# wildjames/lfit_python

Measured on AMD Instinct MI355X. Metric: walker ln_prob evals/sec (300-pt phase, complex BS) at 1/2/4/8 MI355X, higher is better.
Workload: dtype f64

## Files before the change

### cpu_baseline/cpu.py

```python
import ctypes
import os
import subprocess

import numpy as np

HERE = os.path.dirname(os.path.abspath(__file__))
ROOT = os.path.dirname(HERE)
LIB_PATH = os.path.join(HERE, "liblfg_cpu.so")
_dp = ctypes.POINTER(ctypes.c_double)
_ip = ctypes.POINTER(ctypes.c_int)


def build(out=None, march="x86-64-v3"):
    out = out or LIB_PATH
    cmd = ["g++", "-O3", "-march=%s" % march, "-fopenmp", "-std=c++17", "-fPIC", "-shared",
           "-I", HERE, "-I", os.path.join(HERE, "shim"), "-I", os.path.join(ROOT, "lfit_python_amd", "csrc"),
           "-I", os.path.join(ROOT, "include"), "-o", out, os.path.join(HERE, "lfg_cpu.cpp")]
    subprocess.run(cmd, check=True)
    return out


class CpuPort:
    def __init__(self, path=None):
        self.lib = ctypes.CDLL(path or LIB_PATH)
        f = self.lib.lfc_lnprob_batch
        f.restype = ctypes.c_int
        f.argtypes = [_dp, ctypes.c_int, ctypes.c_int, ctypes.c_int, _ip, _ip, _dp, _ip, _dp, _dp, _dp, _dp,
                      ctypes.c_int, _ip, _dp, _dp, _dp, ctypes.c_int, _dp, ctypes.c_int]
        for name in ("lfg_cpu_flux", "lfg_cpu_lnlike", "lfg_cpu_lnprob"):
            getattr(self.lib, name).restype = ctypes.c_int
        self.lib.lfg_cpu_flux.argtypes = [_dp, ctypes.c_int, ctypes.c_int, _dp, _dp, ctypes.c_int, ctypes.c_int,
                                          _dp, _ip, ctypes.c_int]
        self.lib.lfg_cpu_lnlike.argtypes = [_dp, ctypes.c_int, ctypes.c_int, _dp, _dp, ctypes.c_int, ctypes.c_int,
                                            _dp, _dp, _dp, _ip, ctypes.c_int]
        g = self.lib.lfc_lnprob_batch_gp
        g.restype = ctypes.c_int
        g.argtypes = [_dp, ctypes.c_int, ctypes.c_int, ctypes.c_int, _ip, _ip, _dp, _ip, _dp, _dp, _dp, _dp,
                      ctypes.c_int, _ip, _dp, _dp, _dp, ctypes.c_int, _ip, _dp, _ip, _dp, ctypes.c_int]

    def lnprob_batch(self, walkers, tree, nthreads=0):
        keep = []

        def F(a):
            a = np.ascontiguousarray(a, dtype=np.float64)
            keep.append(a)
            return a.ctypes.data_as(_dp)

        def I(a):
            a = np.ascontiguousarray(a, dtype=np.int32)
            keep.append(a)
            return a.ctypes.data_as(_ip)
        w = np.ascontiguousarray(walkers, dtype=np.float64)
        W, ndim = w.shape
        lnp = np.empty(W)
        gp = bool(getattr(tree, "gp", False))
        used = self.lib.lfc_lnprob_batch_gp(
            F(w), W, ndim, tree.E, I(tree.gather.reshape(-1)), I(tree.npars),
            F(tree.consts if len(tree.consts) else np.zeros(1)), I(tree.offsets), F(tree.x), F(tree.y), F(tree.ye),
            F(tree.w), int(tree.nsub), I(tree.prior_type), F(tree.prior_p1), F(tree.prior_p2), F(tree.prior_norm),
            int(tree.roche_priors), I(tree.gp_gather.reshape(-1)) if gp else None,
            F(tree.gp_base.reshape(-1)) if gp else None, I(tree.gp_ecl.reshape(-1)) if gp else None,
            lnp.ctypes.data_as(_dp), int(nthreads))
        if getattr(tree, "fixed_invalid", False):
            lnp[:] = -np.inf
        return lnp, used

    def flux(self, pars, x, w, nsub=1, nthreads=0):
        pars = np.ascontiguousarray(np.atleast_2d(pars), dtype=np.float64)
        x = np.ascontiguousarray(x, dtype=np.float64)
        w = None if w is None else np.ascontiguousarray(w, dtype=np.float64)
        W, P = pars.shape
        flux = np.empty((W, x.size))
        st = np.empty(W, dtype=np.int32)
        rc = self.lib.lfg_cpu_flux(pars.ctypes.data_as(_dp), W, P, x.ctypes.data_as(_dp),
                                   None if w is None else w.ctypes.data_as(_dp), x.size, int(nsub),
                                   flux.ctypes.data_as(_dp), st.ctypes.data_as(_ip), int(nthreads))
        if rc != 0:
            raise ValueError("lfg_cpu_flux: code %d" % rc)
        return flux, st

    def lnlike(self, pars, x, w, y, ye, nsub=1, nthreads=0):
        pars = np.ascontiguousarray(np.atleast_2d(pars), dtype=np.float64)
        arr = [np.ascontiguousarray(a, dtype=np.float64) for a in (x, y, ye)]
        w = None if w is None else np.ascontiguousarray(w, dtype=np.float64)
        W, P = pars.shape
        out = np.empty(W)
        st = np.empty(W, dtype=np.int32)
        rc = self.lib.lfg_cpu_lnlike(pars.ctypes.data_as(_dp), W, P, arr[0].ctypes.data_as(_dp),
                                     None if w is None else w.ctypes.data_as(_dp), arr[0].size, int(nsub),
                                     arr[1].ctypes.data_as(_dp), arr[2].ctypes.data_as(_dp), out.ctypes.data_as(_dp),
                                     st.ctypes.data_as(_ip), int(nthreads))
        if rc != 0:
            raise ValueError("lfg_cpu_lnlike: code %d" % rc)
        return out, st

    def gp_predict(self, x, ye, obs, res, hyp, blocks, return_var=True, nthreads=0):
        x, ye = (np.ascontiguousarray(a, dtype=np.float64).reshape(-1) for a in (x, ye))
        obs = np.ascontiguousarray(obs, dtype=np.int32).reshape(-1)
# ... 48 lines not shown
```

### cpu_baseline/lfg_cpu.cpp

```cpp
#include <omp.h>
#include <stdint.h>
#include <stdlib.h>

#include <algorithm>
#include <cmath>
#include <vector>

#include "lfg.h"
#include "lfg_cpu.h"
#include "lfg_device.hpp"
#include "lfg_tables.hpp"

using namespace lfg;

namespace {

constexpr int U_WD = NWD / 2, U_DISC = NDISC / 2, U_DON = NDONOR / 4;

struct Pair {
    Roche R;
    double s, c, rwd_a, rdisc_a, reff, rcal, ulimb, dexp, L, upk, umax, lnpk, exp1, exp2;
    double bsx, bsy, caz, saz, nb0, nb1, nb2, bden, fis, phi0, wdf, df, sf, rsf;
    double inc;
};
// ... 38 lines not shown
    if (st == ST_OK && (!(p[9] > 0.0) || !(p[14] > 0.0) || !(p[15] > 0.0))) st = ST_BAD_GEOMETRY;
    double bs[4] = {0.0, 0.0, 0.0, 0.0};
    int bst = (std::isfinite(p[6]) && std::isfinite(p[10])) ? bspot<false>(R, G.rdisc_a, bs, &qp) : ST_BAD_ARGS;
    if (bst != ST_OK) {
        rprior = -INFINITY;
    } else {
        double alpha = std::atan2(bs[1], bs[0]) / DEG;
        if (alpha < 0.0) alpha = 90.0 - alpha;
        const double tangent = alpha + 90.0;
        if (p[10] < std::fmax(0.0, tangent - AZ_SLOPE) || p[10] > std::fmin(178.0, tangent + AZ_SLOPE)) rprior = -INFINITY;
    }
    if (st != ST_OK) return st;
    if (bst != ST_OK) return bst;
    const double a1 = p[14], a2 = p[15];
    G.upk = std::pow(a1 / a2, 1.0 / a2);
    G.lnpk = a1 * std::log(G.upk) - std::pow(G.upk, a2);
    G.umax = bs_umax(a1, a2, G.lnpk);
    if (!(std::isfinite(G.upk) && std::isfinite(G.lnpk) && std::isfinite(G.umax))) return ST_BAD_GEOMETRY;
    G.exp1 = a1;
    G.exp2 = a2;
    G.bsx = bs[0];
    G.bsy = bs[1];
    G.s = std::sin(inc * DEG);
    G.c = std::cos(inc * DEG);
    const double tilt = p[16] * DEG, psi = (p[10] - 90.0 + p[17]) * DEG;
    const double st_ = std::sin(tilt), ct_ = std::cos(tilt);
    G.nb0 = st_ * std::cos(psi);
    G.nb1 = st_ * std::sin(psi);
    G.nb2 = ct_;
    G.caz = std::cos(p[10] * DEG);
    G.saz = std::sin(p[10] * DEG);
    G.bden = p[11] + (1.0 - p[11]) * std::fmax(std::fabs(st_) * G.s + ct_ * G.c, 0.0);
    G.fis = p[11];
    G.phi0 = p[13];
    G.ulimb = p[7];
    G.dexp = p[12];
    G.L = p[9] * R.xl1;
    G.reff = eggleton(R.q);
    const double sce = G.s * std::cos(PI * p[5]);
    G.rcal = std::sqrt(1.0 - sce * sce);
    G.wdf = p[0]; G.df = p[1]; G.sf = p[2]; G.rsf = p[3];
    G.inc = inc;
    return ST_OK;
}

struct Tables {
    double a[NWD + NDISC], b[NWD + NDISC], w[NWD + NDISC];
    int wd[NWD + NDISC];
    double sa[NBS], sb[NBS], sw[NBS];
    double dv[NDONOR][3], dcen[NDONOR], dhw[NDONOR];
    double dnorm;
};

#ifdef LFC_COUNT
static unsigned long long g_cnt[4 + 3 * 8];
extern "C" void lfc_counts(unsigned long long* o) { for (int i = 0; i < 4 + 24; ++i) o[i] = g_cnt[i]; }
static unsigned long long g_ucost[U_WD + U_DISC + NBS];
extern "C" void lfc_ucost(unsigned long long* o) { for (int i = 0; i < U_WD + U_DISC + NBS; ++i) { o[i] = g_ucost[i]; g_ucost[i] = 0; } }
static void count_pair(const int* cost, int n)
{
    unsigned long long ls = 0, cm = 0, nc = 0;
    for (int k = 0; k < n; k += 64) {
        int m = 0;
        for (int i = k; i < std::min(n, k + 64); ++i) {
            m = std::max(m, cost[i]);
            ls += cost[i];
            const int reg = i < U_WD ? 0 : (i < U_WD + U_DISC ? 1 : 2);
#pragma omp atomic
            g_ucost[i] += cost[i];
#pragma omp atomic
            g_cnt[4 + reg * 8 + std::min(cost[i], 7)] += 1;
        }
        cm += m; ++nc;
    }
#pragma omp atomic
    g_cnt[0] += n;
#pragma omp atomic
    g_cnt[1] += ls;
#pragma omp atomic
    g_cnt[2] += nc;
#pragma omp atomic
    g_cnt[3] += cm;
}
#define LFC_NIT int nit[3] = {0, 0, 0}; bool fb = false; double gs[2] = {0.0, 0.0};
#define LFC_NITARGS , &fb, nit, gs
#if LFC_COST_MODE == 1
#define LFC_COST(v) cost[v] = nit[0] / 1000
#elif LFC_COST_MODE == 2
#define LFC_COST(v) cost[v] = nit[0] % 1000 + std::max(nit[1], nit[2]) + (fb ? 30 : 0)
#else
#define LFC_COST(v) cost[v] = nit[0] + std::max(nit[1], nit[2]) + (fb ? 30 : 0)
#endif
static std::vector<double> g_ab;
extern "C" long lfc_dump(double* o, long n)
{
    const long m = std::min<long>(n, long(g_ab.size()));
    for (long i = 0; i < m; ++i) o[i] = g_ab[i];
    g_ab.clear();
    return m;
}
#define LFC_AB(a, b) do { _Pragma("omp critical") { g_ab.push_back(a); g_ab.push_back(b); g_gs.push_back(gs[0]); g_gs.push_back(gs[1]); } } while (0)
static std::vector<double> g_gs;
extern "C" long lfc_dump_guess(double* o, long n)
{
    const long m = std::min<long>(n, long(g_gs.size()));
    for (long i = 0; i < m; ++i) o[i] = g_gs[i];
    g_gs.clear();
    return m;
}
#else
#define LFC_NIT
#define LFC_NITARGS
#define LFC_COST(v)
#define LFC_AB(a, b)
#endif

void elements(const Pair& G, Tables& T)
{
#ifdef LFC_COUNT
    int cost[U_WD + U_DISC + NBS] = {0};
#endif
    const Roche& R = G.R;
    const double s = G.s, c = G.c;
    const double twd = TWO_PI * ((1.0 - G.ulimb) * 0.5 + G.ulimb / 3.0);
    const double td = TWO_PI * (disc_boundary(NDISC_R, G) - disc_boundary(0, G));
    int k = 0;
    for (int u = 0; u < U_WD + U_DISC; ++u) {
        double Px, Py, Pz, wgt;
        bool isw = u < U_WD;
        if (isw) {
            const int ir = wd_ring_of(u);
            const double rc = kWdRc[ir], mu0 = kWdMu0[ir], cp = kWdCos[u], sp = kWdSin[u];
            Px = G.rwd_a * (-rc * sp * c + mu0 * s);
            Py = G.rwd_a * (rc * cp);
            Pz = G.rwd_a * (rc * sp * s + mu0 * c);
            wgt = std::fma(kWdA[ir], 1.0 - G.ulimb, kWdB[ir] * G.ulimb) / twd;
        } else {
            const int uu = u - U_WD, ir = uu / (NDISC_AZ / 2), j = uu - ir * (NDISC_AZ / 2);
            const double rc = G.rwd_a + (ir + 0.5) * ((G.rdisc_a - G.rwd_a) / NDISC_R);
            Px = rc * kDiscCos[j];
            Py = rc * kDiscSin[j];
            Pz = 0.0;
            wgt = (TWO_PI / NDISC_AZ) * (disc_boundary(ir + 1, G) - disc_boundary(ir, G)) / td;
        }
        double a, b;
        LFC_NIT
        element_interval_fast(R, Px, Py, Pz, s, c, G.rcal, G.reff, a, b LFC_NITARGS);
        LFC_COST(u);
        LFC_AB(a, b);
        T.a[k] = a; T.b[k] = b; T.w[k] = wgt; T.wd[k] = isw; ++k;
        const bool ecl = a < b;
        T.a[k] = ecl ? -b : 1.0; T.b[k] = ecl ? -a : -1.0; T.w[k] = wgt; T.wd[k] = isw; ++k;
    }
    double tot = 0.0;
    for (int j = 0; j < NBS; ++j) {
        const double uk = (j + 0.5) * (G.umax / NBS);
        T.sw[j] = std::exp(G.exp1 * std::log(uk) - std::pow(uk, G.exp2) - G.lnpk);
        tot += T.sw[j];
        const double off = G.L * (uk - G.upk);
        LFC_NIT
        element_interval_fast(R, std::fma(off, G.caz, G.bsx), std::fma(off, G.saz, G.bsy), 0.0, s, c, G.rcal, G.reff,
                              T.sa[j], T.sb[j] LFC_NITARGS);
        LFC_COST(U_WD + U_DISC + j);
        LFC_AB(T.sa[j], T.sb[j]);
    }
#ifdef LFC_COUNT
    count_pair(cost, U_WD + U_DISC + NBS);
#endif
    for (int j = 0; j < NBS; ++j) T.sw[j] /= tot;
    double dn = 0.0;
    for (int uu = 0; uu < U_DON; ++uu) {
        const int it = uu / (NDONOR_P / 4), ip = uu - it * (NDONOR_P / 4);
        const double dx = -kDonCt[it], dy = kDonSt[it] * kDonCp[ip], dz = kDonSt[it] * kDonSp[ip];
        double lo = 0.0, hi = R.Rs, r = G.reff, gx, gy, gz;
        if (!(r > lo && r < hi)) r = 0.5 * hi;
        for (int itr = 0; itr < ROOT_MAXIT; ++itr) {
            const double f = rpot_grad(R, std::fma(r, dx, 1.0), r * dy, r * dz, gx, gy, gz) - R.pl1;
            const double df = gx * dx + gy * dy + gz * dz;
            if (f > 0.0) hi = r; else lo = r;
            if (df > 0.0 && std::fabs(f / df) <= ROOT_LAST) { r -= f / df; break; }
            double rn = (df > 0.0) ? r - f / df : 0.5 * (lo + hi);
            if (!(rn > lo && rn < hi)) rn = 0.5 * (lo + hi);
            r = rn;
        }
        rgrad(R, std::fma(r, dx, 1.0), r * dy, r * dz, gx, gy, gz);
        const double ig = 1.0 / std::sqrt(gx * gx + gy * gy + gz * gz);
        const double nx = gx * ig, ny = gy * ig, nz = gz * ig;
        const double dA = r * r * kDonOmega[it] / (nx * dx + ny * dy + nz * dz);
        const double vx = dA * nx, vy = dA * ny, vz = dA * nz;
        const double srho = s * std::sqrt(vx * vx + vy * vy);
        const double kap = (srho > 0.0) ? -c * vz / srho : (c * vz > 0.0 ? -2.0 : 2.0);
        const double cen = -std::atan2(vy, vx) / TWO_PI, hw = std::acos(std::fmin(std::fmax(kap, -1.0), 1.0)) / TWO_PI;
        for (int mr = 0; mr < 4; ++mr) {
            const int t = 4 * uu + mr;
            T.dv[t][0] = vx;
            T.dv[t][1] = (mr & 1) ? -vy : vy;
            T.dv[t][2] = (mr & 2) ? -vz : vz;
            T.dcen[t] = (mr & 1) ? -cen : cen;
            T.dhw[t] = (mr & 2) ? 0.5 - hw : hw;
            dn += std::fmax(-s * T.dv[t][1] + c * T.dv[t][2], 0.0);
        }
    }
    T.dnorm = dn;
}

double wrap_phase(double ph) { return ph - std::floor(ph + 0.5); }

void sweep_window(const double* lo, const double* hi, const double* iw, int m, double a, double b, double wn,
                  double* d, double* direct)
{
    const int P2 = int(std::lower_bound(lo, lo + m, a) - lo);
    const int P4 = int(std::lower_bound(lo, lo + m, b) - lo);
    const int P1 = int(std::upper_bound(hi, hi + m, a) - hi);
    const int P3 = int(std::upper_bound(hi, hi + m, b) - hi);
    int e0 = P4, s1 = P4;
    if (P2 < P3) {
        d[P2] += wn;
        d[P3] -= wn;
        e0 = P2;
        s1 = P3;
    }
    for (int r = 0; r < 2; ++r)
        for (int p = r ? s1 : P1; p < (r ? P4 : e0); ++p) {
            if (hi[p] > lo[p]) {
                const double ov = std::fmin(b, hi[p]) - std::fmax(a, lo[p]);
                if (ov > 0.0) direct[p] += wn * ov * iw[p];
            } else if (a < lo[p] && lo[p] < b) {
                direct[p] += wn;
            }
        }
}

void sweep_points(const double* ph, int m, double x1, double x2, const double* v, std::vector<double>& d3)
{
    const int P = int(std::upper_bound(ph, ph + m, x1) - ph), Q = int(std::lower_bound(ph, ph + m, x2) - ph);
    if (P < Q)
        for (int k = 0; k < 3; ++k) {
            d3[3 * P + k] += v[k];
            d3[3 * Q + k] -= v[k];
        }
}

double chisq(const Pair& G, const Tables& T, const double* x, const double* w, const double* y, const double* ye, int n,
             int S, std::vector<double>& buf, double* fout = nullptr)
{
    const int ns = n * S;
    buf.assign(size_t(9) * n + size_t(10) * ns + 8, 0.0);
    double* lo = buf.data();
    double* hi = lo + n;
    double* iw = hi + n;
    double* dw = iw + n;
    double* dd = dw + n + 1;
    double* xw = dd + n + 1;
    double* xd = xw + n;
    double* slo = xd + n + 1;
    double* shi = slo + ns;
    double* siw = shi + ns;
    double* sph = siw + ns;
    double* ds = sph + ns;
// ... 353 lines not shown
```

### cpu_baseline/shim/hip/hip_runtime.h

```cpp
#pragma once
#include <algorithm>
#include <cmath>
#define __device__
#define __host__
#define __global__
#define __constant__
#define __forceinline__ inline
#define __noinline__
#define __builtin_amdgcn_rsq(x) (1.0 / std::sqrt(x))
#define __builtin_amdgcn_rcp(x) (1.0 / (x))
using std::max;
using std::min;
inline double rsqrt(double x) { return 1.0 / std::sqrt(x); }
inline float rsqrtf(float x) { return 1.0f / std::sqrt(x); }
```

### lfit_python_amd/csrc/lfg.hip

```cpp
#include <hip/hip_runtime.h>
#include <atomic>
#include <stdint.h>
#include <stdlib.h>

#include <type_traits>

#include "lfg.h"
#include "lfg_device.hpp"
#include "lfg_tables.hpp"

using namespace lfg;

#if defined(LFG_PROFILE_PAIR) || defined(LFG_COUNT_ITERS) || defined(LFG_COUNT_QUIET)
#define LFG_ONE_TU 1
#endif

namespace {

constexpr int SETUP_BLOCK = 64;
#ifndef LFG_ELEM_BLOCK
#define LFG_ELEM_BLOCK 64
#endif
constexpr int ELEM_BLOCK = LFG_ELEM_BLOCK;
#ifndef LFG_ELEM_IPL
// ... 520 lines not shown
template <typename GPtr>
__device__ __forceinline__ void ring_weight_lane(int rb, GPtr G, double* __restrict__ wtd)
{
    const double P = disc_boundary(rb, G);
    const int lane = int(threadIdx.x) & 63, l0 = lane - rb;
    const double Pn = __shfl(P, min(lane + 1, l0 + NDISC_R), 64);
    const double Pt = __shfl(P, l0 + NDISC_R, 64);
    if (rb < NDISC_R) wtd[rb] = (TWO_PI / NDISC_AZ) * (Pn - P);
    if (rb == 0) wtd[NDISC_R] = TWO_PI * (Pt - P);
}

template <typename GPtr, typename Sink>
__device__ __forceinline__ void element_item_to(int v, GPtr G, Sink& K);

struct MemSink {
    const ElemOut& O;
    __device__ __forceinline__ void mark() {}
    __device__ __forceinline__ void wd_disc(int u, double a, double b) { O.abw[uslot(u)] = make_double2(a, b); }
    __device__ __forceinline__ void spot(int j, double a, double b, double w)
    {
        O.abs[j] = make_double2(a, b);
        O.wbs[j] = w;
    }
    __device__ __forceinline__ void donor(int uu, double vx, double vy, double vz, double cen, double hw)
    {
        double* D = O.don + uu * DON_STRIDE;
        D[0] = vx;
        D[1] = vy;
        D[2] = vz;
        D[3] = cen;
        D[4] = hw;
    }
};

template <typename GPtr>
__device__ __forceinline__ void element_item(int v, GPtr G, const ElemOut& O)
{
    MemSink K{O};
    element_item_to(v, G, K);
}

__device__ __forceinline__ void element_lane(int v, int pair, int npairs, const double* __restrict__ G, int st0, int bst,
                                             int* status, double2* __restrict__ AB, double* __restrict__ DON,
                                             double* __restrict__ WT, const ElemSpec& X)
{
    double* Wp = WT + size_t(pair) * WT_N;
    if (v >= NUNIQ) {
        const int rb = v - NUNIQ;
        if (rb > NDISC_R || st0 != ST_OK) return;
        ring_weight_lane(rb, G, Wp + WT_DISC);
        return;
    }
    static_assert((NUNIQ % ELEM_BLOCK) + NDISC_R + 1 <= ELEM_BLOCK, "ring-weight lanes fit in the last chunk");
    static_assert(WT_TD == WT_DISC + NDISC_R, "disc total follows the ring weights");
    if (st0 != ST_OK) return;
    if (bst != ST_OK) {
        if (v == 0 && !X.jk) status[pair] = bst;
        return;
    }
    if (X.lprior) {
        const int w = pair / X.E;
        const double lp = X.jk ? X.priorC[size_t(X.accflag[X.jk[w]]) * (npairs / X.E) + w] : X.lprior[w];
        if (prior_rejects(lp, G)) return;
    }
    double2* ABp = AB + size_t(pair) * NELU;
    element_item(v, G, ElemOut{ABp, ABp + NU_WDD, DON + size_t(pair) * U_DON * DON_STRIDE, Wp + WT_DISC, Wp + WT_BS});
}

template <typename GPtr, typename Sink>
__device__ __forceinline__ void element_item_to(int v, GPtr G, Sink& K)
{
    constexpr int V_BS = U_WD + U_DISC;
    const int u = (v < V_BS) ? v : (v < V_BS + U_BS ? U_MAIN + (v - V_BS) : v - U_BS);
    const Roche R{G[G_Q], G[G_CA], G[G_CB], G[G_MU], G[G_XL1], G[G_PL1], G[G_RS], G[G_RS2]};
    const double s = G[G_S], c = G[G_C];

    if (u >= U_WD + U_DISC && u < U_MAIN) {
        const int uu = u - (U_WD + U_DISC);
        const int it = uu / (NDONOR_P / 4), ip = uu - it * (NDONOR_P / 4);
        const double stc = kDonSt[it], ctc = kDonCt[it];
        const double dx = -ctc, dy = stc * kDonCp[ip], dz = stc * kDonSp[ip];
        double lo = 0.0, hi = R.Rs, r = G[G_REFF];
        if (!(r > lo && r < hi)) r = 0.5 * hi;
        double gx, gy, gz;
        for (int itr = 0; itr < ROOT_MAXIT; ++itr) {
            const double X0 = fma(r, dx, 1.0), X1 = r * dy, X2 = r * dz;
            const double f = rpot_grad(R, X0, X1, X2, gx, gy, gz) - R.pl1;
            const double df = gx * dx + gy * dy + gz * dz;
            if (f > 0.0) hi = r; else lo = r;
            const double stp = f * rcp_fast(df);
            if (df > 0.0 && fabs(stp) <= ROOT_LAST) { r -= stp; break; }
            double rn = (df > 0.0) ? r - stp : 0.5 * (lo + hi);
            if (!(rn > lo && rn < hi)) rn = 0.5 * (lo + hi);
            r = rn;
        }
        rgrad(R, fma(r, dx, 1.0), r * dy, r * dz, gx, gy, gz);
        const double ig = rsqrt(gx * gx + gy * gy + gz * gz);
        const double nx = gx * ig, ny = gy * ig, nz = gz * ig;
        const double dA = r * r * kDonOmega[it] / (nx * dx + ny * dy + nz * dz);
        const double vx = dA * nx, vy = dA * ny, vz = dA * nz;
        const double srho = s * sqrt(vx * vx + vy * vy);
        const double kap = (srho > 0.0) ? -c * vz / srho : (c * vz > 0.0 ? -2.0 : 2.0);
        const double cen = -atan2(vy, vx) * (1.0 / TWO_PI), hw = acos(fmin(fmax(kap, -1.0), 1.0)) * (1.0 / TWO_PI);
        K.mark();
        K.donor(uu, vx, vy, vz, cen, hw);
        return;
    }

    double Px, Py, Pz;
    if (u < U_WD) {
        const int ir = wd_ring_of(u);
        const double rc = kWdRc[ir], mu0 = kWdMu0[ir];
        const double cp = kWdCos[u], sp = kWdSin[u];
        const double rw = G[G_RWD];
        Px = rw * (-rc * sp * c + mu0 * s);
        Py = rw * (rc * cp);
        Pz = rw * (rc * sp * s + mu0 * c);
    } else if (u < U_WD + U_DISC) {
        const int uu = u - U_WD;
        const int ir = uu / (NDISC_AZ / 2), j = uu - ir * (NDISC_AZ / 2);
        const double rin = G[G_RWD];
        const double rc = rin + (ir + 0.5) * ((G[G_RDISC] - rin) / NDISC_R);
        Px = rc * kDiscCos[j];
        Py = rc * kDiscSin[j];
        Pz = 0.0;
    } else {
        const int j = u - U_MAIN;
        const double uk = (j + 0.5) * (G[G_UMAX] / NBS);
        const double off = G[G_L] * (uk - G[G_UPK]);
        Px = fma(off, G[G_CAZ], G[G_BSX]);
        Py = fma(off, G[G_SAZ], G[G_BSY]);
        Pz = 0.0;
    }
    double a, b;
#ifdef LFG_COUNT_ITERS
    bool fb = false;
    int nit[3] = {0, 0, 0};
    double gs[2] = {0.0, 0.0};
    element_interval_fast(R, Px, Py, Pz, s, c, G[G_RCAL], G[G_REFF], a, b, &fb, nit, gs);
    {
        const int reg = (u < U_WD) ? 0 : (u < U_WD + U_DISC ? 1 : 2);
        unsigned long long* C = g_iter_dbg + reg * 16;
        for (int i = 0; i < 3; ++i) {
            atomicAdd(C + i, (unsigned long long)nit[i]);
            int m = nit[i];
            for (int off = 32; off > 0; off >>= 1) m = max(m, __shfl_xor(m, off, 64));
            if ((threadIdx.x & 63) == 0) atomicAdd(C + 3 + i, (unsigned long long)m);
        }
        if ((threadIdx.x & 63) == 0) atomicAdd(C + 9, 1ull);
        atomicAdd(C + 6, fb ? 1ull : 0ull);
        if (fb) {
            const unsigned long long k = atomicAdd(g_iter_dbg + 48, 1ull);
            if (k < 15) g_iter_dbg[49 + k] = (static_cast<unsigned long long>(blockIdx.x) << 16) | unsigned(u);
        }
        atomicAdd(C + 7, 1ull);
        atomicAdd(C + 8, (a < b) ? 1ull : 0ull);
        if (a < b && !fb) {
            const double er = fmax(fabs(gs[0] - a * TWO_PI), fabs(gs[1] - b * TWO_PI));
            const int bin = er < 1e-4 ? 0 : er < 1e-3 ? 1 : er < 1e-2 ? 2 : er < 3e-2 ? 3 : er < 1e-1 ? 4 : 5;
            atomicAdd(C + 10 + bin, 1ull);
        }
    }
#else
    element_interval_fast(R, Px, Py, Pz, s, c, G[G_RCAL], G[G_REFF], a, b);
#endif
    K.mark();
    if (u >= U_MAIN) K.spot(u - U_MAIN, a, b, bs_weight(u - U_MAIN, G));
    else K.wd_disc(u, a, b);
}

#ifdef LFG_PROFILE_ELEM
__device__ unsigned long long g_elem_wav[4][32768];
__device__ __forceinline__ void elem_stamp(unsigned long long t0, int kind)
{
    if ((threadIdx.x & 63) == 0 && blockIdx.x < 32768) {
        unsigned hw;
        asm volatile("s_getreg_b32 %0, hwreg(HW_REG_HW_ID)" : "=s"(hw));
        g_elem_wav[0][blockIdx.x] = t0;
        g_elem_wav[1][blockIdx.x] = __builtin_amdgcn_s_memrealtime();
        g_elem_wav[2][blockIdx.x] = hw;
        g_elem_wav[3][blockIdx.x] = kind;
    }
}
#endif

#ifndef LFG_NOLICM_TU
__global__ __launch_bounds__(ELEM_BLOCK) __attribute__((amdgpu_waves_per_eu(ELEM_MINW))) void k_elements(const double* __restrict__ geo, int* status, int npairs,
                                                         double2* __restrict__ AB, double* __restrict__ DON,
                                                         double* __restrict__ WT, const int* __restrict__ bstatus,
                                                         ElemSpec X)
{
#ifdef LFG_PROFILE_ELEM
    const unsigned long long pt0 = __builtin_amdgcn_s_memrealtime();
#endif
    if (int(blockIdx.x) < X.nspecblk) {
        const int nb = (X.nspec + int(blockDim.x) - 1) / int(blockDim.x);
        const int c = int(blockIdx.x) < nb ? 0 : 1;
        const int t = (int(blockIdx.x) - c * nb) * int(blockDim.x) + int(threadIdx.x);
        if (t < X.nspec) setup_any(X.S[__builtin_amdgcn_readfirstlane(c)], t);
#ifdef LFG_PROFILE_ELEM
        elem_stamp(pt0, 0);
#endif
        return;
    }
    const unsigned bid = blockIdx.x - unsigned(X.nspecblk);
    const int pair = int(bid % unsigned(npairs));
    static_assert(ELEM_BLOCK * LFG_ELEM_IPL == 64 && (NUNIQ + NDISC_R + 1 + 63) / 64 == 15, "chunk order table");
    constexpr int kOrder[15] = {13, 14, 12, 11, 10, 9, 8, 7, 6, 5, 4, 3, 2, 1, 0};
    const int ck = kOrder[bid / unsigned(npairs)];
    const int v0 = ck * (int(blockDim.x) * LFG_ELEM_IPL) + int(threadIdx.x);
    const double* G = geo + size_t(pair) * LFG_NGEO;
    int st0, bst;
    if (X.jk) {
        const int w = pair / X.E, e = pair - w * X.E;
        const size_t cp = size_t(X.accflag[X.jk[w]]) * npairs + pair;
        G = X.geoC + cp * LFG_NGEO;
        st0 = X.statusC[cp];
        bst = X.bstatusC[cp];
        if (bid < unsigned(npairs)) {
            const int l = int(threadIdx.x);
            double* Gd = const_cast<double*>(geo) + size_t(pair) * LFG_NGEO;
            if (l < LFG_NGEO) Gd[l] = G[l];
            if (l == LFG_NGEO) status[pair] = (st0 != ST_OK) ? st0 : bst;
            if (l == LFG_NGEO + 1) X.bstatus[pair] = bst;
            if (e == 0) {
                const size_t cw = size_t(X.accflag[X.jk[w]]) * (npairs / X.E) + w;
                for (int d = l; d < X.ndim; d += int(blockDim.x)) X.q[size_t(w) * X.ndim + d] = X.qC[cw * X.ndim + d];
                if (l == LFG_NGEO + 2) X.prior[w] = X.priorC[cw];
// ... 4426 lines not shown
```

### lfit_python_amd/csrc/lfg_device.hpp

```cpp
#pragma once
#include <hip/hip_runtime.h>
#include <math.h>

#include "lfg_stream_table.h"

namespace lfg {

constexpr double PI = 3.14159265358979323846;
constexpr double TWO_PI = 6.28318530717958647693;
constexpr double DEG = PI / 180.0;
constexpr double LN2 = 0.69314718055994530942;

constexpr double RAY_TOL = 1e-13;
constexpr int RAY_MAXIT = 100;
constexpr double TH_TOL = 1e-13;
constexpr int ROOT_MAXIT = 100;
constexpr double ROOT_LAST = 1e-9;
constexpr int MIN_MAXIT = 100;
constexpr double BS_TAIL = 16.0;
constexpr double STREAM_DELTA = 1e-2;
constexpr double STREAM_KAPPA_FINE = 0.15 / 32.0;
constexpr double STREAM_DTMAX_FINE = 0.15 / 32.0;
constexpr int STREAM_MAXSTEP_FINE = 128000;
constexpr double DISC_MAX_A = 0.46;
// ... 274 lines not shown
            }
            double tn = (chord && have && dg != pdg) ? th - dg * (th - pth) / (dg - pdg)
                                                     : 0.5 * (mlo + mhi);
            if (!(tn > mlo && tn < mhi)) tn = 0.5 * (mlo + mhi);
            if (fabs(tn - th) <= TH_TOL) break;
            if (chord) { pth = th; pdg = dg; have = true; }
            th = tn;
            chord = g_eval(R, Px, Py, Pz, s, c, th, tw, g, dg);
        }
        if (!found) return false;
    }
    double de;
    const double ce = (sqrt(fmax(uu - Reff * Reff, 0.0)) - c * uz) / (s * uxy);
    de = (ce > -1.0 && ce < 1.0) ? acos(ce) : 0.5 * Dm;
    double twi = tw, two = tw;
    const double thin = theta_root(R, Px, Py, Pz, s, c, lo, thi, true, thc - de, twi);
    const double thout = theta_root(R, Px, Py, Pz, s, c, thi, hi, false, thc + de, two);
    a = thin * (1.0 / TWO_PI);
    b = thout * (1.0 / TWO_PI);
    return true;
}

struct ConePt {
    double phi, gth, F2, eHe, etHe, ethHeth, gtt, dX2;
};

__device__ __forceinline__ void cone_point(const Roche& R, double Px, double Py, double Pz, double s,
                                           double c, double cs, double sn, double t, ConePt& o)
{
    const double ex = s * cs, ey = -s * sn;
    const double x = fma(t, ex, Px), y = fma(t, ey, Py), z = fma(t, c, Pz);
    const double r1s = x * x + y * y + z * z;
    const double ir1 = rsqrt_pos(r1s), ir1s = ir1 * ir1;
    const double dx = x - 1.0;
    const double r2s = dx * dx + y * y + z * z;
    const double ir2 = rsqrt_pos(r2s), ir2s = ir2 * ir2;
    const double i1 = R.cA * ir1s * ir1, i2 = R.cB * ir2s * ir2, i12 = i1 + i2;
    const double xm = x - R.mu;
    o.phi = -R.cA * ir1 - R.cB * ir2 - xm * xm - y * y;
    const double gx = i1 * x + i2 * dx - 2.0 * xm;
    const double gy = (i12 - 2.0) * y;
    const double gz = i12 * z;
    const double p1 = x * ex + y * ey + z * c, p2 = p1 - ex;
    const double q1 = x * ey - y * ex, q2 = q1 - ey;
    const double k1 = 3.0 * i1 * ir1s, k2 = 3.0 * i2 * ir2s;
    const double s2 = ex * ex + ey * ey;
    o.F2 = gx * ex + gy * ey + gz * c;
    o.gth = gx * ey - gy * ex;
    o.eHe = i12 - k1 * p1 * p1 - k2 * p2 * p2 - 2.0 * s2;
    o.etHe = -k1 * p1 * q1 - k2 * p2 * q2;
    o.ethHeth = i12 * s2 - k1 * q1 * q1 - k2 * q2 * q2 - 2.0 * s2;
    o.gtt = -(gx * ex + gy * ey);
    o.dX2 = r2s;
}

__device__ __forceinline__ void rotate(double& cs, double& sn, double d)
{
    const double d2 = d * d;
    const double sd = d * (1.0 - d2 * (1.0 / 6.0) * (1.0 - d2 * (1.0 / 20.0) * (1.0 - d2 * (1.0 / 42.0) *
                                                                              (1.0 - d2 * (1.0 / 72.0)))));
    const double cd = 1.0 - d2 * 0.5 * (1.0 - d2 * (1.0 / 12.0) * (1.0 - d2 * (1.0 / 30.0) *
                                                                    (1.0 - d2 * (1.0 / 56.0) * (1.0 - d2 * (1.0 / 90.0)))));
    const double c2 = cs * cd - sn * sd;
    sn = fma(sn, cd, cs * sd);
    cs = c2;
}

#ifndef LFG_TH_LAST
#define LFG_TH_LAST 1e-6
#endif
#ifndef LFG_T_LAST
#define LFG_T_LAST 3e-5
#endif
constexpr double TH_LAST = LFG_TH_LAST;
constexpr double T_LAST = LFG_T_LAST;

struct Tan {
    double th, cs, sn, t;
    int st;
};

template <bool HALLEY = false>
__device__ __forceinline__ void tangency_step(const Roche& R, double Px, double Py, double Pz, double s, double c,
                                              bool ingress, Tan& T)
{
    ConePt o;
    cone_point(R, Px, Py, Pz, s, c, T.cs, T.sn, T.t, o);
    const double F1 = o.phi - R.pl1;
    const double J11 = T.t * o.gth;
    const double J21 = T.t * o.etHe + o.gth, J22 = o.eHe;
    const double iJ22 = rcp_step(J22);
    const double dt0 = -o.F2 * iJ22;
    const double F1m = fma(0.5 * o.F2, dt0, F1);
    const double den = fma(J21, dt0, J11);
    const bool bad = !(J22 != 0.0) || !(den != 0.0);
    const double iden = rcp_step(den);
    double dth = -F1m * iden;
    if (HALLEY) {
        const double g2 = fma(T.t, fma(T.t, o.ethHeth, o.gtt), -J21 * J21 * iJ22);
        const double h = 0.5 * dth * g2 * iden;
        if (fabs(h) < 0.5) dth = dth * rcp_step(1.0 + h);
    }
    dth = fmin(fmax(dth, -0.05), 0.05);
    const double dt = fma(-J21 * iJ22, dth, dt0);
    T.th += dth;
    T.t += dt;
    const bool conv = fabs(dth) <= TH_LAST && fabs(dt) <= T_LAST;
    const bool good = J22 > 0.0 && ((J11 < 0.0) == ingress) && T.t > 0.0 && o.dX2 < R.Rs2;
    rotate(T.cs, T.sn, dth);
    T.st = bad ? -1 : (conv ? (good ? 1 : -1) : 0);
}

__device__ inline bool tangency(const Roche& R, double Px, double Py, double Pz, double s, double c,
                                bool ingress, double& th, double cs, double sn, double& t, int* nit = nullptr)
{
    Tan T{th, cs, sn, t, 0};
    for (int it = 0; it < 16 && T.st == 0; ++it) {
        if (nit) ++*nit;
        tangency_step(R, Px, Py, Pz, s, c, ingress, T);
    }
    th = T.th;
    t = T.t;
    return T.st == 1;
}

__device__ inline void tangency_pair(const Roche& R, double Px, double Py, double Pz, double s, double c, Tan& A,
                                     Tan& B, int* nit = nullptr)
{
    tangency_step<true>(R, Px, Py, Pz, s, c, true, A);
    tangency_step<true>(R, Px, Py, Pz, s, c, false, B);
    if (nit) { nit[0] += 1; nit[1] += 1; }
    if (A.st != 0 && B.st != 0) return;
    for (int it = 1; it < 16; ++it) {
        Tan A2 = A, B2 = B;
        tangency_step(R, Px, Py, Pz, s, c, true, A2);
        tangency_step(R, Px, Py, Pz, s, c, false, B2);
        if (nit) { nit[0] += (A.st == 0); nit[1] += (B.st == 0); }
        if (A.st == 0) A = A2;
        if (B.st == 0) B = B2;
        if (A.st != 0 && B.st != 0) break;
    }
}

__device__ inline int cone_exists(const Roche& R, double Px, double Py, double Pz, double s, double c,
                                  double cs, double sn, double t, int* nit = nullptr)
{
    for (int it = 0; it < 16; ++it) {
        if (nit) ++*nit;
        ConePt o;
        cone_point(R, Px, Py, Pz, s, c, cs, sn, t, o);
        if (o.phi < R.pl1) return (o.dX2 < R.Rs2) ? 1 : -1;
        const double Gth = t * o.gth, Gt = o.F2;
        const double Htt = o.eHe, Hht = o.gth + t * o.etHe, Hhh = t * t * o.ethHeth + t * o.gtt;
        const double det = Hhh * Htt - Hht * Hht;
        if (!(Hhh > 0.0 && Htt > 0.0 && det > 0.0)) return -1;
        const double idet = rcp_fast(det);
        double dth = -(Htt * Gth - Hht * Gt) * idet;
        double dt = -(Hhh * Gt - Hht * Gth) * idet;
        const double big = fmax(fabs(dth), fabs(dt));
        if (big > 0.05) {
            dth *= 0.05 / big;
            dt *= 0.05 / big;
        }
        t += dt;
        if (fabs(dth) <= 1e-12 && fabs(dt) <= 1e-12) return 0;
        rotate(cs, sn, dth);
    }
    return -1;
}

__device__ inline bool element_interval_fast(const Roche& R, double Px, double Py, double Pz, double s,
                                             double c, double Rcal, double Reff, double& a, double& b,
                                             bool* fallback = nullptr, int* nit = nullptr, double* guess = nullptr)
{
    const double ux = 1.0 - Px, uy = -Py, uz = -Pz;
    const double uxy2 = ux * ux + uy * uy;
    const double uu = uxy2 + uz * uz;
    if (uu > R.Rs2 && uxy2 > 0.0 && s > 0.0) {
        const double iuxy = rsqrt(uxy2), uxy = uxy2 * iuxy;
        const double cosD = (sqrt(uu - R.Rs2) - c * uz) * iuxy / s;
        if (!(cosD < 1.0)) { a = 1.0; b = -1.0; return false; }
        const double cc = ux * iuxy, sc = -uy * iuxy;
        const double tc = s * uxy + uz * c;
        int ex;
        {
            const double ex0 = s * cc, ey0 = -s * sc;
            const double x = fma(tc, ex0, Px), y = fma(tc, ey0, Py), z = fma(tc, c, Pz);
            const double dx = x - 1.0, xm = x - R.mu;
            const double r2s = dx * dx + y * y + z * z;
            const double phi = -R.cA * rsqrt_pos(x * x + y * y + z * z) - R.cB * rsqrt_pos(r2s) - xm * xm - y * y;
            if (phi < R.pl1 && r2s < R.Rs2) {
                ex = 1;
                if (nit) ++nit[0];
            } else {
                ex = cone_exists(R, Px, Py, Pz, s, c, cc, sc, tc, nit);
            }
        }
        if (ex == 0) { a = 1.0; b = -1.0; return false; }
        if (ex == 1) {
            const double ce = (sqrt(fmax(uu - Rcal * Rcal, 0.0)) - c * uz) * iuxy / s;
            if (ce > -1.0 && ce < 1.0) {
                const double se = sqrt(1.0 - ce * ce);
                const double thc = atan2(-uy, ux), de = acos(ce);
                double ci = cc * ce + sc * se, si = sc * ce - cc * se;
                double co = cc * ce - sc * se, so = sc * ce + cc * se;
                Tan In{thc - de, ci, si, s * (ux * ci - uy * si) + uz * c, 0};
                Tan Out{thc + de, co, so, s * (ux * co - uy * so) + uz * c, 0};
                if (guess) { guess[0] = In.th; guess[1] = Out.th; }
                {
                    const double icb = R.cB / (Rcal * Rcal * Rcal) - 2.0 * s * s;
                    for (Tan* T : {&In, &Out}) {
                        const double ex = s * T->cs, ey = -s * T->sn;
                        const double x = fma(T->t, ex, Px), y = fma(T->t, ey, Py), z = fma(T->t, c, Pz);
                        const double ir1 = rsqrt_pos(x * x + y * y + z * z), ir1s = ir1 * ir1;
                        const double eX = x * ex + y * ey + z * c;
                        const double i1 = R.cA * ir1s * ir1;
                        const double slope = fma(i1, eX, -2.0 * fma(x - R.mu, ex, y * ey));
                        const double curv = fma(i1, fma(-3.0 * eX * eX, ir1s, 1.0), icb);
                        T->t -= slope * rcp_fast(curv);
                    }
                }
                tangency_pair(R, Px, Py, Pz, s, c, In, Out, nit ? nit + 1 : nullptr);
                const double cin = In.cs * cc + In.sn * sc, cout = Out.cs * cc + Out.sn * sc;
                if (In.st == 1 && Out.st == 1 && In.th < Out.th && cin > cosD && cout > cosD) {
                    a = In.th * (1.0 / TWO_PI);
                    b = Out.th * (1.0 / TWO_PI);
                    return true;
                }
            }
        }
    }
    if (fallback) *fallback = true;
    return element_interval(R, Px, Py, Pz, s, c, Reff, a, b);
}

__device__ inline int findphi(const Roche& R, double inc_deg, double& dphi);

__device__ inline int findphi_fast(const Roche& R, double inc_deg, double& dphi)
{
    double s, c;
    sincos(inc_deg * DEG, &s, &c);
    const double cosD = sqrt(1.0 - R.Rs2) / s;
    if (s > 0.0 && cosD < 1.0) {
        const double Dm = acos(cosD);
        const double R0 = eggleton(R.q);
        const double c0 = sqrt(1.0 - R0 * R0) / s;
        double th = (c0 < 1.0) ? acos(c0) : 0.5 * Dm;
        double sn, cs;
        sincos(th, &sn, &cs);
        double t = s * cs;
        if (tangency(R, 0.0, 0.0, 0.0, s, c, false, th, cs, sn, t) && th > 0.0 && th < Dm) {
            dphi = th / PI;
            return ST_OK;
        }
    }
    return findphi(R, inc_deg, dphi);
}

__device__ inline int findphi(const Roche& R, double inc_deg, double& dphi)
{
    const double i = inc_deg * DEG;
    double s, c;
    sincos(i, &s, &c);
    dphi = 0.0;
    const double cosD = sqrt(1.0 - R.Rs2) / s;
    if (!(s > 0.0) || cosD >= 1.0) return ST_BAD_DPHI;
    const double Dm = acos(cosD);
    double tw = -1.0, g, dg;
    g_eval(R, 0.0, 0.0, 0.0, s, c, 0.0, tw, g, dg);
    if (!(g < 0.0)) return ST_BAD_DPHI;
    const double th = theta_root(R, 0.0, 0.0, 0.0, s, c, 0.0, Dm, false, 0.5 * Dm, tw);
    dphi = th / PI;
    return ST_OK;
}

__device__ inline bool h_eval(const Roche& R, double cth, double sth, double c,
                              double& tw, double& h, double& dh)
{
    const double s = sqrt(1.0 - c * c);
    const double ex = s * cth, ey = -s * sth;
    double fm;
    if (!ray_min(R, 0.0, 0.0, 0.0, ex, ey, c, tw, fm)) { h = 1.0; dh = 0.0; return false; }
    double gx, gy, gz;
    rgrad(R, tw * ex, tw * ey, tw * c, gx, gy, gz);
    h = fm - R.pl1;
    const double r = c / s;
    dh = tw * (gx * (-r * cth) + gy * (r * sth) + gz);
    return true;
}

__device__ inline int findi(const Roche& R, double dphi, double& inc_deg)
{
    if (!(dphi > 0.0) || !(dphi < 0.5)) return ST_BAD_DPHI;
    const double the = PI * dphi;
    double sth, cth;
    sincos(the, &sth, &cth);
    if (!(cth > 0.0)) return ST_BAD_DPHI;
    const double smin = sqrt(1.0 - R.Rs2) / cth;
    if (smin >= 1.0) return ST_BAD_DPHI;
    const double cmax = sqrt(1.0 - smin * smin);
    double tw = -1.0, h, dh;
    h_eval(R, cth, sth, 0.0, tw, h, dh);
    if (!(h < 0.0)) return ST_BAD_DPHI;
    double lo = 0.0, hi = cmax, c = 0.5 * cmax;
    for (int it = 0; it < ROOT_MAXIT; ++it) {
// ... 536 lines not shown
```

Measured before the change: 13.49 million.

## Warm-start tangency Newton solve with packed FP32 iterations before FP64 refinement

Adds an FP32 packed-pair (two-lane vector) Newton/Halley pre-solve for ingress and egress tangency points, with validity checks that fall back to the original FP64 ray-minimum prestep. When the FP32 warm start succeeds, the first FP64 tangency step uses plain Newton instead of Halley. This aims to cut the number of costly FP64 iterations on MI355X by moving the early convergence work to cheaper FP32 math. The risk is accuracy loss or extra branching when the FP32 guesses fail. An optional FP32 root pre-solve and CPU counters are also added, but the root pre-solve is off by default.

```diff
diff --git a/cpu_baseline/cpu.py b/cpu_baseline/cpu.py
--- a/cpu_baseline/cpu.py
+++ b/cpu_baseline/cpu.py
@@ -11,9 +11,9 @@
 _ip = ctypes.POINTER(ctypes.c_int)
 
 
-def build(out=None, march="x86-64-v3"):
+def build(out=None, march="x86-64-v3", extra=()):
     out = out or LIB_PATH
-    cmd = ["g++", "-O3", "-march=%s" % march, "-fopenmp", "-std=c++17", "-fPIC", "-shared",
+    cmd = ["g++", "-O3", "-march=%s" % march, "-fopenmp", "-std=c++17", "-fPIC", "-shared"] + list(extra) + [
            "-I", HERE, "-I", os.path.join(HERE, "shim"), "-I", os.path.join(ROOT, "lfit_python_amd", "csrc"),
            "-I", os.path.join(ROOT, "include"), "-o", out, os.path.join(HERE, "lfg_cpu.cpp")]
     subprocess.run(cmd, check=True)
diff --git a/cpu_baseline/lfg_cpu.cpp b/cpu_baseline/lfg_cpu.cpp
--- a/cpu_baseline/lfg_cpu.cpp
+++ b/cpu_baseline/lfg_cpu.cpp
@@ -144,14 +144,19 @@
 #pragma omp atomic
     g_cnt[3] += cm;
 }
+static unsigned long long g_cnt2[5];
+extern "C" void lfc_counts2(unsigned long long* o) { for (int i = 0; i < 5; ++i) o[i] = g_cnt2[i]; }
+static void count2(int i, unsigned long long v)
+{
+#pragma omp atomic
+    g_cnt2[i] += v;
+}
 #define LFC_NIT int nit[3] = {0, 0, 0}; bool fb = false; double gs[2] = {0.0, 0.0};
 #define LFC_NITARGS , &fb, nit, gs
 #if LFC_COST_MODE == 1
 #define LFC_COST(v) cost[v] = nit[0] / 1000
-#elif LFC_COST_MODE == 2
-#define LFC_COST(v) cost[v] = nit[0] % 1000 + std::max(nit[1], nit[2]) + (fb ? 30 : 0)
 #else
-#define LFC_COST(v) cost[v] = nit[0] + std::max(nit[1], nit[2]) + (fb ? 30 : 0)
+#define LFC_COST(v) cost[v] = nit[0] % 1000 + std::max(nit[1], nit[2]) + (fb ? 30 : 0); count2(0, nit[0] / 1000); count2(1, fb)
 #endif
 static std::vector<double> g_ab;
 extern "C" long lfc_dump(double* o, long n)
@@ -236,7 +241,17 @@
         const double dx = -kDonCt[it], dy = kDonSt[it] * kDonCp[ip], dz = kDonSt[it] * kDonSp[ip];
         double lo = 0.0, hi = R.Rs, r = G.reff, gx, gy, gz;
         if (!(r > lo && r < hi)) r = 0.5 * hi;
+#if LFG_F32_OPEN && LFG_F32_ROOT_STEPS > 0
+        r = root_open32<LFG_F32_ROOT_STEPS>(R, dx, dy, dz, hi, r);
+#endif
+#ifdef LFC_COUNT
+        count2(2, 1);
+        count2(4, LFG_F32_OPEN ? LFG_F32_ROOT_STEPS : 0);
+#endif
         for (int itr = 0; itr < ROOT_MAXIT; ++itr) {
+#ifdef LFC_COUNT
+            count2(3, 1);
+#endif
             const double f = rpot_grad(R, std::fma(r, dx, 1.0), r * dy, r * dz, gx, gy, gz) - R.pl1;
             const double df = gx * dx + gy * dy + gz * dz;
             if (f > 0.0) hi = r; else lo = r;
diff --git a/cpu_baseline/shim/hip/hip_runtime.h b/cpu_baseline/shim/hip/hip_runtime.h
--- a/cpu_baseline/shim/hip/hip_runtime.h
+++ b/cpu_baseline/shim/hip/hip_runtime.h
@@ -9,6 +9,8 @@
 #define __noinline__
 #define __builtin_amdgcn_rsq(x) (1.0 / std::sqrt(x))
 #define __builtin_amdgcn_rcp(x) (1.0 / (x))
+#define __builtin_amdgcn_rsqf(x) (1.0f / std::sqrt(float(x)))
+#define __builtin_amdgcn_rcpf(x) (1.0f / float(x))
 using std::max;
 using std::min;
 inline double rsqrt(double x) { return 1.0 / std::sqrt(x); }
diff --git a/lfit_python_amd/csrc/lfg.hip b/lfit_python_amd/csrc/lfg.hip
--- a/lfit_python_amd/csrc/lfg.hip
+++ b/lfit_python_amd/csrc/lfg.hip
@@ -626,6 +626,9 @@
         const double dx = -ctc, dy = stc * kDonCp[ip], dz = stc * kDonSp[ip];
         double lo = 0.0, hi = R.Rs, r = G[G_REFF];
         if (!(r > lo && r < hi)) r = 0.5 * hi;
+#if LFG_F32_OPEN && LFG_F32_ROOT_STEPS > 0
+        r = root_open32<LFG_F32_ROOT_STEPS>(R, dx, dy, dz, hi, r);
+#endif
         double gx, gy, gz;
         for (int itr = 0; itr < ROOT_MAXIT; ++itr) {
             const double X0 = fma(r, dx, 1.0), X1 = r * dy, X2 = r * dz;
@@ -686,8 +689,9 @@
         const int reg = (u < U_WD) ? 0 : (u < U_WD + U_DISC ? 1 : 2);
         unsigned long long* C = g_iter_dbg + reg * 16;
         for (int i = 0; i < 3; ++i) {
-            atomicAdd(C + i, (unsigned long long)nit[i]);
-            int m = nit[i];
+            const int ni = i ? nit[i] : nit[0] % 1000;
+            atomicAdd(C + i, (unsigned long long)ni);
+            int m = ni;
             for (int off = 32; off > 0; off >>= 1) m = max(m, __shfl_xor(m, off, 64));
             if ((threadIdx.x & 63) == 0) atomicAdd(C + 3 + i, (unsigned long long)m);
         }
diff --git a/lfit_python_amd/csrc/lfg_device.hpp b/lfit_python_amd/csrc/lfg_device.hpp
--- a/lfit_python_amd/csrc/lfg_device.hpp
+++ b/lfit_python_amd/csrc/lfg_device.hpp
@@ -380,7 +380,7 @@
 
 template <bool HALLEY = false>
 __device__ __forceinline__ void tangency_step(const Roche& R, double Px, double Py, double Pz, double s, double c,
-                                              bool ingress, Tan& T)
+                                              bool ingress, Tan& T, bool halley = true)
 {
     ConePt o;
     cone_point(R, Px, Py, Pz, s, c, T.cs, T.sn, T.t, o);
@@ -394,7 +394,7 @@
     const bool bad = !(J22 != 0.0) || !(den != 0.0);
     const double iden = rcp_step(den);
     double dth = -F1m * iden;
-    if (HALLEY) {
+    if (HALLEY && halley) {
         const double g2 = fma(T.t, fma(T.t, o.ethHeth, o.gtt), -J21 * J21 * iJ22);
         const double h = 0.5 * dth * g2 * iden;
         if (fabs(h) < 0.5) dth = dth * rcp_step(1.0 + h);
@@ -423,10 +423,10 @@
 }
 
 __device__ inline void tangency_pair(const Roche& R, double Px, double Py, double Pz, double s, double c, Tan& A,
-                                     Tan& B, int* nit = nullptr)
-{
-    tangency_step<true>(R, Px, Py, Pz, s, c, true, A);
-    tangency_step<true>(R, Px, Py, Pz, s, c, false, B);
+                                     Tan& B, int* nit = nullptr, bool halleyA = true, bool halleyB = true)
+{
+    tangency_step<true>(R, Px, Py, Pz, s, c, true, A, halleyA);
+    tangency_step<true>(R, Px, Py, Pz, s, c, false, B, halleyB);
     if (nit) { nit[0] += 1; nit[1] += 1; }
     if (A.st != 0 && B.st != 0) return;
     for (int it = 1; it < 16; ++it) {
@@ -439,6 +439,169 @@
         if (A.st != 0 && B.st != 0) break;
     }
 }
+
+__device__ __forceinline__ void ray_min_prestep(const Roche& R, double Px, double Py, double Pz, double s, double c,
+                                                double icb, Tan& T)
+{
+    const double ex = s * T.cs, ey = -s * T.sn;
+    const double x = fma(T.t, ex, Px), y = fma(T.t, ey, Py), z = fma(T.t, c, Pz);
+    const double ir1 = rsqrt_pos(x * x + y * y + z * z), ir1s = ir1 * ir1;
+    const double eX = x * ex + y * ey + z * c;
+    const double i1 = R.cA * ir1s * ir1;
+    const double slope = fma(i1, eX, -2.0 * fma(x - R.mu, ex, y * ey));
+    const double curv = fma(i1, fma(-3.0 * eX * eX, ir1s, 1.0), icb);
+    T.t -= slope * rcp_fast(curv);
+}
+
+#ifndef LFG_F32_OPEN
+#define LFG_F32_OPEN 1
+#endif
+#ifndef LFG_F32_STEPS
+#define LFG_F32_STEPS 2
+#endif
+#ifndef LFG_F32_NEWTON_AFTER
+#define LFG_F32_NEWTON_AFTER 1
+#endif
+#ifndef LFG_F32_ROOT_STEPS
+#define LFG_F32_ROOT_STEPS 0
+#endif
+
+#if LFG_F32_OPEN
+constexpr float F32_OPEN_MIN_WIDTH = 0.03f;
+#ifdef __HIP__
+typedef float F2 __attribute__((ext_vector_type(2)));
+#else
+struct F2 {
+    float x, y;
+};
+inline F2 operator+(F2 a, F2 b) { return F2{a.x + b.x, a.y + b.y}; }
+inline F2 operator-(F2 a, F2 b) { return F2{a.x - b.x, a.y - b.y}; }
+inline F2 operator*(F2 a, F2 b) { return F2{a.x * b.x, a.y * b.y}; }
+inline F2 operator-(F2 a) { return F2{-a.x, -a.y}; }
+#endif
+__device__ __forceinline__ F2 f2(float a) { return F2{a, a}; }
+__device__ __forceinline__ F2 f2_rsq(F2 a) { return F2{__builtin_amdgcn_rsqf(a.x), __builtin_amdgcn_rsqf(a.y)}; }
+__device__ __forceinline__ F2 f2_rcp(F2 a) { return F2{__builtin_amdgcn_rcpf(a.x), __builtin_amdgcn_rcpf(a.y)}; }
+
+template <int N>
+__device__ __forceinline__ void tangency_open32(const Roche& R, double Px, double Py, double Pz, double s, double c,
+                                                double Rcal, Tan& A, Tan& B, bool& okA, bool& okB)
+{
+    float dA, dB, tA, tB;
+    okA = okB = true;
+    {
+        const float cA = float(R.cA), cB = float(R.cB), mu = float(R.mu), pl1 = float(R.pl1);
+        const F2 px = f2(float(Px)), py = f2(float(Py)), pz = f2(float(Pz)), sf = f2(float(s)), cf = f2(float(c));
+        const float rc = float(Rcal);
+        const F2 icb = f2(cB * __builtin_amdgcn_rcpf(rc * rc * rc)) - f2(2.0f) * sf * sf;
+        F2 cs{float(A.cs), float(B.cs)}, sn{float(A.sn), float(B.sn)}, t{float(A.t), float(B.t)};
+        F2 sum = f2(0.0f);
+        {
+            const F2 ex = sf * cs, ey = -(sf * sn);
+            const F2 x = t * ex + px, y = t * ey + py, z = t * cf + pz;
+            const F2 ir1 = f2_rsq(x * x + y * y + z * z), ir1s = ir1 * ir1;
+            const F2 eX = x * ex + y * ey + z * cf;
+            const F2 i1 = f2(cA) * ir1s * ir1;
+            const F2 slope = i1 * eX - f2(2.0f) * ((x - f2(mu)) * ex + y * ey);
+            const F2 curv = i1 * (f2(1.0f) - f2(3.0f) * eX * eX * ir1s) + icb;
+            t = t - slope * f2_rcp(curv);
+        }
+#pragma unroll
+        for (int k = 0; k < N; ++k) {
+            const F2 ex = sf * cs, ey = -(sf * sn);
+            const F2 x = t * ex + px, y = t * ey + py, z = t * cf + pz;
+            const F2 yz = y * y + z * z;
+            const F2 ir1 = f2_rsq(x * x + yz), ir1s = ir1 * ir1;
+            const F2 dx = x - f2(1.0f);
+            const F2 ir2 = f2_rsq(dx * dx + yz), ir2s = ir2 * ir2;
+            const F2 i1 = f2(cA) * ir1s * ir1, i2 = f2(cB) * ir2s * ir2, i12 = i1 + i2;
+            const F2 xm = x - f2(mu);
+            const F2 F1 = -(f2(cA) * ir1) - f2(cB) * ir2 - xm * xm - y * y - f2(pl1);
+            const F2 gx = i1 * x + i2 * dx - f2(2.0f) * xm;
+            const F2 gy = (i12 - f2(2.0f)) * y;
+            const F2 gz = i12 * z;
+            const F2 p1 = x * ex + y * ey + z * cf, p2 = p1 - ex;
+            const F2 q1 = x * ey - y * ex, q2 = q1 - ey;
+            const F2 k1 = f2(3.0f) * i1 * ir1s, k2 = f2(3.0f) * i2 * ir2s;
+            const F2 s2 = ex * ex + ey * ey;
+            const F2 Ft = gx * ex + gy * ey + gz * cf;
+            const F2 gth = gx * ey - gy * ex;
+            const F2 J22 = i12 - k1 * p1 * p1 - k2 * p2 * p2 - f2(2.0f) * s2;
+            const F2 etHe = -(k1 * p1 * q1) - k2 * p2 * q2;
+            const F2 J11 = t * gth, J21 = t * etHe + gth;
+            const F2 iJ22 = f2_rcp(J22);
+            const F2 dt0 = -(Ft * iJ22);
+            const F2 F1m = f2(0.5f) * Ft * dt0 + F1;
+            const F2 iden = f2_rcp(J21 * dt0 + J11);
+            F2 dth = -(F1m * iden);
+            if (k == 0) {
+                const F2 ethHeth = i12 * s2 - k1 * q1 * q1 - k2 * q2 * q2 - f2(2.0f) * s2;
+                const F2 gtt = -(gx * ex + gy * ey);
+                const F2 g2 = t * (t * ethHeth + gtt) - J21 * J21 * iJ22;
+                const F2 h = f2(0.5f) * dth * g2 * iden;
+                const F2 dh = dth * f2_rcp(f2(1.0f) + h);
+                dth = F2{fabsf(h.x) < 0.5f ? dh.x : dth.x, fabsf(h.y) < 0.5f ? dh.y : dth.y};
+            }
+            okA = okA && J22.x > 0.0f && fabsf(dth.x) <= 0.05f;
+            okB = okB && J22.y > 0.0f && fabsf(dth.y) <= 0.05f;
+            t = t + (dt0 - J21 * iJ22 * dth);
+            sum = sum + dth;
+            const F2 d2 = dth * dth;
+            const F2 sd = dth * (f2(1.0f) - d2 * f2(1.0f / 6.0f) * (f2(1.0f) - d2 * f2(1.0f / 20.0f)));
+            const F2 cd = f2(1.0f) - d2 * f2(0.5f) * (f2(1.0f) - d2 * f2(1.0f / 12.0f) *
+                                                                  (f2(1.0f) - d2 * f2(1.0f / 30.0f)));
+            const F2 c2 = cs * cd - sn * sd;
+            sn = sn * cd + cs * sd;
+            cs = c2;
+        }
+        const bool wide = float(B.th - A.th) + (sum.y - sum.x) >= F32_OPEN_MIN_WIDTH;
+        okA = okA && wide && fabsf(sum.x) <= 0.05f && t.x > 0.0f && t.x < 3.0e38f;
+        okB = okB && wide && fabsf(sum.y) <= 0.05f && t.y > 0.0f && t.y < 3.0e38f;
+        dA = okA ? sum.x : 0.0f;
+        dB = okB ? sum.y : 0.0f;
+        tA = t.x;
+        tB = t.y;
+    }
+    A.th += double(dA);
+    B.th += double(dB);
+    rotate(A.cs, A.sn, double(dA));
+    rotate(B.cs, B.sn, double(dB));
+    A.t = double(tA);
+    B.t = double(tB);
+    if (!(okA && okB)) {
+        const double icb = R.cB / (Rcal * Rcal * Rcal) - 2.0 * s * s;
+        for (int k = 0; k < 2; ++k) {
+            Tan& T = k ? B : A;
+            if (k ? okB : okA) continue;
+            T.t = s * ((1.0 - Px) * T.cs + Py * T.sn) - Pz * c;
+            ray_min_prestep(R, Px, Py, Pz, s, c, icb, T);
+        }
+    }
+}
+
+template <int N>
+__device__ __forceinline__ double root_open32(const Roche& R, double dx, double dy, double dz, double hi, double r0)
+{
+    const float cA = float(R.cA), cB = float(R.cB), mu = float(R.mu), pl1 = float(R.pl1);
+    const float ax = float(dx), ay = float(dy), az = float(dz), top = float(hi);
+    float r = float(r0);
+    bool ok = true;
+#pragma unroll
+    for (int k = 0; k < N; ++k) {
+        const float x = fmaf(r, ax, 1.0f), y = r * ay, z = r * az, x1 = r * ax;
+        const float yz = y * y + z * z;
+        const float ir1 = __builtin_amdgcn_rsqf(x * x + yz), ir2 = __builtin_amdgcn_rsqf(x1 * x1 + yz);
+        const float i1 = cA * ir1 * ir1 * ir1, i2 = cB * ir2 * ir2 * ir2;
+        const float xm = x - mu;
+        const float f = -cA * ir1 - cB * ir2 - xm * xm - y * y - pl1;
+        const float gx = i1 * x + i2 * x1 - 2.0f * xm, gy = (i1 + i2 - 2.0f) * y, gz = (i1 + i2) * z;
+        const float df = gx * ax + gy * ay + gz * az;
+        r -= f * __builtin_amdgcn_rcpf(df);
+        ok = ok && df > 0.0f && r > 0.0f && r < top;
+    }
+    return ok ? double(r) : r0;
+}
+#endif
 
 __device__ inline int cone_exists(const Roche& R, double Px, double Py, double Pz, double s, double c,
                                   double cs, double sn, double t, int* nit = nullptr)
@@ -505,20 +668,22 @@
                 Tan In{thc - de, ci, si, s * (ux * ci - uy * si) + uz * c, 0};
                 Tan Out{thc + de, co, so, s * (ux * co - uy * so) + uz * c, 0};
                 if (guess) { guess[0] = In.th; guess[1] = Out.th; }
+#if LFG_F32_OPEN
+                bool openIn, openOut;
+                tangency_open32<LFG_F32_STEPS>(R, Px, Py, Pz, s, c, Rcal, In, Out, openIn, openOut);
+                if (nit) nit[0] += 1000 * LFG_F32_STEPS;
+                const bool hIn = !(LFG_F32_NEWTON_AFTER && openIn), hOut = !(LFG_F32_NEWTON_AFTER && openOut);
+#else
                 {
                     const double icb = R.cB / (Rcal * Rcal * Rcal) - 2.0 * s * s;
-                    for (Tan* T : {&In, &Out}) {
-                        const double ex = s * T->cs, ey = -s * T->sn;
-                        const double x = fma(T->t, ex, Px), y = fma(T->t, ey, Py), z = fma(T->t, c, Pz);
-                        const double ir1 = rsqrt_pos(x * x + y * y + z * z), ir1s = ir1 * ir1;
-                        const double eX = x * ex + y * ey + z * c;
-                        const double i1 = R.cA * ir1s * ir1;
-                        const double slope = fma(i1, eX, -2.0 * fma(x - R.mu, ex, y * ey));
-                        const double curv = fma(i1, fma(-3.0 * eX * eX, ir1s, 1.0), icb);
-                        T->t -= slope * rcp_fast(curv);
-                    }
+                    for (Tan* T : {&In, &Out}) ray_min_prestep(R, Px, Py, Pz, s, c, icb, *T);
                 }
+#endif
+#if LFG_F32_OPEN
+                tangency_pair(R, Px, Py, Pz, s, c, In, Out, nit ? nit + 1 : nullptr, hIn, hOut);
+#else
                 tangency_pair(R, Px, Py, Pz, s, c, In, Out, nit ? nit + 1 : nullptr);
+#endif
                 const double cin = In.cs * cc + In.sn * sc, cout = Out.cs * cc + Out.sn * sc;
                 if (In.st == 1 && Out.st == 1 && In.th < Out.th && cin > cosD && cout > cosD) {
                     a = In.th * (1.0 / TWO_PI);
```

Result: faster. 14.16 million, median of 6 (+5.0%).
